# neoyinyao/Recommender

Hardware: AMD Instinct MI355X
Metric: examples/sec fwd+bwd, Criteo-DLRM 26×40M×128 batch 65536, 1/2/4/8 GPU (higher is better)
Workload: dtype fp32; 1 GPU; dlrm_criteo_26x40000000x128; global_batch=65536, per_gpu_batch=65536, rows=40000000, dim=128, slots=26, optimizer=sgd, parallelism=single, prefetch=False

## Files before the change

### recommender_amd/csrc/interaction.hip

```cpp
#include <map>
#include <mutex>
#include <tuple>
#include <type_traits>

#include "dlrm_shared.hpp"
#include "mfma_x3.hpp"

namespace rs {

struct InterMode {
  int self_interaction;
  int skip_gather;
};

__device__ __forceinline__ bool keep_pair(int i, int j, int self_i) {
  return self_i ? (i >= j) : (i < j);
}

struct GatherSrc {
  const float* table;
  int64_t n_rows;
  const void* ids;
  int32_t id_dtype;
  int32_t n_slots;
// ... 406 lines not shown
  const float* cur = row_of(first, raw_id(first));
  int64_t id_next = raw_id(first + 1);
#pragma unroll
  for (int s = 0; s < KS; ++s) load_rows(cur, s);
  load_g(first, lane);
  float* gs = gsm[wave];
  if (lane == 0) gs[ZS] = 0.f;
  for (int64_t b = first; b < last; ++b) {
    int lanev;
    asm volatile("v_mbcnt_lo_u32_b32 %0, -1, 0\n\tv_mbcnt_hi_u32_b32 %0, -1, %0" : "=v"(lanev));
    const int r = lanev & 31, h = lanev >> 5;
#pragma unroll
    for (int j = 0; j < GREG; ++j) gs[lane + 64 * j] = gnx[j];
    const float* nxt = row_of(b + 1, id_next);
    id_next = raw_id(b + 2);
    __builtin_amdgcn_s_waitcnt(0xc07f);
    __builtin_amdgcn_wave_barrier();
    float sa[KS];
#pragma unroll
    for (int s = 0; s < KS; ++s) {
      const int k = 2 * s + h;
      const bool in = r < F && k < F;
      const bool p1 = in && keep_pair(r, k, SELF);
      const bool p2 = in && keep_pair(k, r, SELF);
      const int j1 = p1 ? (SKIP ? r * F + k : compact_index(r, k, F, SELF)) : ZS;
      const int j2 = p2 ? (SKIP ? k * F + r : compact_index(k, r, F, SELF)) : ZS;
      sa[s] = gs[j1] + gs[j2];
    }
    f32x16 acc[NTILE];
#pragma unroll
    for (int c = 0; c < NTILE; ++c)
#pragma unroll
      for (int e = 0; e < 16; ++e) acc[c][e] = 0.f;
#pragma unroll
    for (int s = 0; s < KS; ++s) {
#pragma unroll
      for (int c = 0; c < NTILE; ++c)
        acc[c] = __builtin_amdgcn_mfma_f32_32x32x2f32(sa[s], xv[s][c], acc[c], 0, 0, 0);
    }
    __builtin_amdgcn_sched_barrier(0);
#pragma unroll
    for (int s = 0; s < KS; ++s) load_rows(nxt, s);
    __builtin_amdgcn_sched_barrier(0);
    float dpass[NTILE];
#pragma unroll
    for (int c = 0; c < NTILE; ++c) dpass[c] = gs[nz + NTILE * r + c];
    load_g(b + 1, lanev);
#pragma unroll
    for (int reg = 0; reg < 16; ++reg) {
      const int i = (reg & 3) + 8 * (reg >> 2) + 4 * h;
      if (i < F) {
        float v[NTILE];
#pragma unroll
        for (int c = 0; c < NTILE; ++c) v[c] = acc[c][reg] + (i == S ? dpass[c] : 0.f);
        float* dst = (i < S ? gemb + (b * S + i) * (int64_t)D : gdense + b * D) + NTILE * r;
        *reinterpret_cast<float4*>(dst) = make_float4(v[0], v[1], v[2], v[3]);
      }
    }
  }
  if (__any(oob) && lane == 0) flag_oob(src.err_flag);
}

constexpr int kDxLdx = 136;
constexpr int kDxRows = 28;
constexpr int kDxZt = 32 * 33;

template <bool ID64>
__global__ __launch_bounds__(256) void dlrm_fwd_dx_pipe(GatherSrc src, int64_t batch, int F,
                                                        float* __restrict__ out,
                                                        int64_t out_stride, FwdHead hd, int epw) {
  constexpr int D = 128, NT = 8;
  __shared__ __attribute__((aligned(16))) float lds[4][kDxRows * kDxLdx + kDxZt];
  const int wave = threadIdx.x >> 6, lane = threadIdx.x & 63;
  const int64_t first = ((int64_t)blockIdx.x * 4 + wave) * epw;
  if (first >= batch) return;
  const int64_t last = first + epw < batch ? first + epw : batch;
  const int r = lane & 15, g = lane >> 4;
  const int r32 = lane & 31, h = lane >> 5;
  const int S = src.n_slots;
  const int nzc = F * (F - 1) / 2;
  float* X = lds[wave];
  float(*z)[33] = reinterpret_cast<float(*)[33]>(lds[wave] + kDxRows * kDxLdx);
  float qz[8], qd[2], sa[2][8], qdn[4];
#pragma unroll
  for (int t = 0; t < 8; ++t) qz[t] = lane + 64 * t < nzc ? hd.q[lane + 64 * t] : 0.f;
#pragma unroll
  for (int t = 0; t < 2; ++t) qd[t] = hd.q[nzc + lane + 64 * t];
  const float cc = hd.c[0];
#pragma unroll
  for (int ib = 0; ib < 2; ++ib)
#pragma unroll
    for (int kk = 0; kk < 8; ++kk) {
      const int m = 16 * ib + r, k = 4 * kk + g;
      const bool in = m < F && k < F && m != k;
      const float v = hd.q[in ? compact_index(m < k ? m : k, m < k ? k : m, F, 0) : 0];
      sa[ib][kk] = in ? v : 0.f;
    }
#pragma unroll
  for (int c = 0; c < 4; ++c) qdn[c] = hd.q[nzc + 4 * r32 + c];
  int zoff[8];
#pragma unroll
  for (int t = 0; t < 8; ++t) {
    const int o = lane + 64 * t;
    int i = 0, j = 0;
    if (o < nzc) compact_pair(o, F, false, i, j);
    zoff[t] = o < nzc ? i * 33 + j : -1;
  }
  int64_t lo = 0, n_ok = src.n_rows;
  if (lane < S && src.slot_offsets) {
    lo = src.slot_offsets[lane];
    n_ok = src.slot_offsets[lane + 1] - lo;
  }
  bool oob = false;
  auto raw_id = [&](int64_t b) -> int64_t {
    const int64_t bb = b < last ? b : first;
    const int ln = lane < S ? lane : S - 1;
    const int64_t v = ID64 ? static_cast<const int64_t*>(src.ids)[bb * S + ln]
                           : static_cast<int64_t>(static_cast<const int32_t*>(src.ids)[bb * S + ln]);
    return lane < S ? v : 0;
  };
  auto row_of = [&](int64_t b, int64_t id) -> const float* {
    const bool live = b < last;
    const bool id_ok = id >= 0 && id < n_ok;
    if (lane < S && !id_ok && live) oob = true;
    if (lane < S) return id_ok ? src.table + (lo + id) * D : kZeroRow;
    return (lane == S && live) ? src.dense + (b < last ? b : first) * D : kZeroRow;
  };
  f4 a0[NT], a1[NT];
  float dnv[2];
  auto gather = [&](const float* mine, int64_t b) {
    const float* p0 = shfl_ptr(mine, r);
    const float* p1 = shfl_ptr(mine, 16 + r);
#pragma unroll
    for (int t = 0; t < NT; ++t) {
      a0[t] = *(gfloatx4*)(p0 + 4 * g + 16 * t);
      a1[t] = *(gfloatx4*)(p1 + 4 * g + 16 * t);
    }
    const int64_t bb = b < last ? b : first;
#pragma unroll
    for (int t = 0; t < 2; ++t) dnv[t] = *(gfloat*)(src.dense + bb * D + lane + 64 * t);
  };
  gather(row_of(first, raw_id(first)), first);
  int64_t id_next = raw_id(first + 1);
  for (int64_t b = first; b < last; ++b) {
    int lanev;
    asm volatile("v_mbcnt_lo_u32_b32 %0, -1, 0\n\tv_mbcnt_hi_u32_b32 %0, -1, %0" : "=v"(lanev));
    const int r = lanev & 15, g = (lanev >> 4) & 3;
    const int r32 = lanev & 31, h = (lanev >> 5) & 1;
    const float* nxt = row_of(b + 1, id_next);
    id_next = raw_id(b + 2);
    f4 c00 = {0.f, 0.f, 0.f, 0.f}, c01 = c00, c11 = c00;
#pragma unroll
    for (int t = 0; t < NT; ++t) {
#pragma unroll
      for (int c = 0; c < 4; ++c) {
        c00 = __builtin_amdgcn_mfma_f32_16x16x4f32(a0[t][c], a0[t][c], c00, 0, 0, 0);
        c01 = __builtin_amdgcn_mfma_f32_16x16x4f32(a0[t][c], a1[t][c], c01, 0, 0, 0);
        c11 = __builtin_amdgcn_mfma_f32_16x16x4f32(a1[t][c], a1[t][c], c11, 0, 0, 0);
      }
    }
#pragma unroll
    for (int t = 0; t < NT; ++t) {
      *reinterpret_cast<f4*>(&X[r * kDxLdx + 16 * t + 4 * g]) = a0[t];
      if (16 + r < kDxRows) *reinterpret_cast<f4*>(&X[(16 + r) * kDxLdx + 16 * t + 4 * g]) = a1[t];
    }
    float dn_cur[2] = {dnv[0], dnv[1]};
    __builtin_amdgcn_sched_barrier(0);
    gather(nxt, b + 1);
    __builtin_amdgcn_sched_barrier(0);
#pragma unroll
    for (int reg = 0; reg < 4; ++reg) {
      const int i = 4 * g + reg;
      z[i][r] = c00[reg];
      z[i][16 + r] = c01[reg];
      z[16 + r][i] = c01[reg];
      z[16 + i][16 + r] = c11[reg];
    }
    __builtin_amdgcn_wave_barrier();
    float* orow = out + b * out_stride;
    float hacc = 0.f;
    const int pad = nzc + D;
#pragma unroll
    for (int t = 0; t < 8; ++t) {
      const int o = lanev + 64 * t;
      const bool in = zoff[t] >= 0;
      const float v = in ? (&z[0][0])[zoff[t]] : 0.f;
      orow[in ? o : pad] = v;
      hacc += v * qz[t];
    }
    float* od = orow + nzc;
#pragma unroll
    for (int t = 0; t < 2; ++t) {
      const int d = lanev + 64 * t;
      od[d] = dn_cur[t];
      hacc += dn_cur[t] * qd[t];
    }
#pragma unroll
    for (int off = 32; off > 0; off >>= 1) hacc += __shfl_xor(hacc, off);
    {
      const float v = hacc + cc;
      hd.y[b] = hd.act == 2 ? 1.f / (1.f + expf(-v)) : (hd.act == 1 ? fmaxf(v, 0.f) : v);
    }
    {
      const int o = pad + lanev;
      orow[o < out_stride ? o : pad] = 0.f;
    }
#pragma unroll
    for (int t = 0; t < NT; ++t) {
      constexpr int KK = kDxRows / 4;
      float bv[KK];
#pragma unroll
      for (int kk = 0; kk < KK; ++kk) bv[kk] = X[(4 * kk + g) * kDxLdx + 16 * t + r];
      f4 d0 = {0.f, 0.f, 0.f, 0.f}, d1 = d0;
#pragma unroll
      for (int kk = 0; kk < KK; ++kk) {
        d0 = __builtin_amdgcn_mfma_f32_16x16x4f32(sa[0][kk], bv[kk], d0, 0, 0, 0);
        d1 = __builtin_amdgcn_mfma_f32_16x16x4f32(sa[1][kk], bv[kk], d1, 0, 0, 0);
      }
#pragma unroll
      for (int reg = 0; reg < 4; ++reg) {
        const int i0 = 4 * g + reg, i1 = 16 + 4 * g + reg;
        X[i0 * kDxLdx + 16 * t + r] = d0[reg];
        if (i1 < kDxRows) X[i1 * kDxLdx + 16 * t + r] = d1[reg];
      }
    }
    __builtin_amdgcn_wave_barrier();
    float* de = hd.dxu_emb + b * S * (int64_t)D;
#pragma unroll
    for (int s2 = 0; s2 < kDxRows / 2; ++s2) {
      const int i = 2 * s2 + h < S ? 2 * s2 + h : S;
      f4 v = *reinterpret_cast<const f4*>(&X[i * kDxLdx + 4 * r32]);
      const bool emb = i < S;
#pragma unroll
      for (int c = 0; c < 4; ++c) v[c] = emb ? v[c] : v[c] + qdn[c];
      float* dst = emb ? de + i * D : hd.dxu_dense + b * D;
      *reinterpret_cast<f4*>(dst + 4 * r32) = v;
    }
    __builtin_amdgcn_wave_barrier();
  }
  if (__any(oob) && lane == 0) flag_oob(src.err_flag);
}

__device__ __forceinline__ void split3(const f4& lo, const f4& hi, bf8& h, bf8& m,
                                       bf8& l) {
#pragma unroll
  for (int j = 0; j < 4; ++j) {
    bf2 hp, mp, lp;
    split_pair(j < 2 ? f2{lo[2 * j], lo[2 * j + 1]} : f2{hi[2 * j - 4], hi[2 * j - 3]}, hp, mp, lp);
    h[2 * j] = hp[0];
    h[2 * j + 1] = hp[1];
    m[2 * j] = mp[0];
    m[2 * j + 1] = mp[1];
    l[2 * j] = lp[0];
    l[2 * j + 1] = lp[1];
  }
}

constexpr int kTrainAtop = 512;
constexpr int kTrainNI = 13;
template <int D>
constexpr int train_m() { return kTrainAtop + 2 + kTrainNI * D + D; }
constexpr int kTrainM = train_m<128>();

struct TrainArgs {
  const float* q;
  const float* c;
  const float* label;
  const float* xin;
  float eps;
  float gscale;
  float* y;
  float* grad_emb;
  float* part;
};

typedef short shortx4 __attribute__((ext_vector_type(4)));
typedef short shortx8 __attribute__((ext_vector_type(8)));
typedef __attribute__((address_space(3))) shortx4 lds_shortx4;

__device__ __forceinline__ f4 mfma6_xs(const bf8& xh, const bf8& xm, const bf8& xl,
                                            const bf8& sh, const bf8& sm, const bf8& sl,
                                            f4 c) {
  c = __builtin_amdgcn_mfma_f32_16x16x32_bf16(xm, sm, c, 0, 0, 0);
  c = __builtin_amdgcn_mfma_f32_16x16x32_bf16(xl, sh, c, 0, 0, 0);
  c = __builtin_amdgcn_mfma_f32_16x16x32_bf16(xh, sl, c, 0, 0, 0);
  c = __builtin_amdgcn_mfma_f32_16x16x32_bf16(xm, sh, c, 0, 0, 0);
  c = __builtin_amdgcn_mfma_f32_16x16x32_bf16(xh, sm, c, 0, 0, 0);
  return __builtin_amdgcn_mfma_f32_16x16x32_bf16(xh, sh, c, 0, 0, 0);
}

constexpr int kChPlane = 32 * 32 * 2;
constexpr int kChImage = 3 * kChPlane;
__device__ __forceinline__ int ch_off(int row, int col) {
  const int chunk = (col >> 3) ^ ((row >> 1) & 3) ^ (((row >> 3) & 1) << 1);
  return row * 64 + 16 * chunk + 2 * (col & 7);
}
constexpr int kChStageLd = 36;
template <int D>
constexpr int chunk_region_floats() {
  return (kChImage / 4 + 32 * kChStageLd + D) > train_m<D>() ? (kChImage / 4 + 32 * kChStageLd + D)
                                                             : train_m<D>();
}

template <int D, bool ID64>
__global__ __launch_bounds__(256, 2) void dlrm_train_chunk(GatherSrc src, int64_t batch, int F,
                                                        TrainArgs ta, float* g_rows, int epw) {
  static_assert(D == 64 || D == 128, "train kernel laid out for D = 64 or 128");
  constexpr int NT = D / 16, NC = D / 32, DL = D / 4, RPI = 64 / DL, DPL = D / 64;
  constexpr int TM = train_m<D>();
  constexpr int RW = chunk_region_floats<D>();
  __shared__ __attribute__((aligned(16))) float lds[4][RW];
  __shared__ __attribute__((aligned(16))) float qlane[64][12];
  __shared__ __attribute__((aligned(16))) float qsh[kTrainAtop];
  __shared__ __attribute__((aligned(16))) bf8 sash[2][3][64];
  const int wave = threadIdx.x >> 6, lane = threadIdx.x & 63;
  const int64_t first = ((int64_t)blockIdx.x * 4 + wave) * epw;
  const int64_t last = first + epw < batch ? first + epw : batch;
  const bool active = first < batch;
  const int r = lane & 15, g = lane >> 4;
  const int S = src.n_slots;
  const int nzc = F * (F - 1) / 2;
  char* img = reinterpret_cast<char*>(lds[wave]);
  float* stg = lds[wave] + kChImage / 4;
  float* ubot = stg + 32 * kChStageLd;
  for (int e = threadIdx.x; e < kTrainAtop; e += 256) {
    const float v = ta.q[e < nzc + D ? e : 0];
    qsh[e] = e < nzc + D ? v : 0.f;
  }
  if (wave == 0) {
    float qv[12];
    bool qk[12];
#pragma unroll
    for (int reg = 0; reg < 4; ++reg) {
      const int i0 = 4 * g + reg, j0 = r;
      const int i1 = 4 * g + reg, j1 = 16 + r;
      const int i2 = 16 + 4 * g + reg, j2 = 16 + r;
      qk[reg] = i0 < j0 && j0 < F;
      qk[4 + reg] = j1 < F;
      qk[8 + reg] = i2 < j2 && j2 < F;
      qv[reg] = ta.q[qk[reg] ? compact_index(i0, j0, F, 0) : 0];
      qv[4 + reg] = ta.q[qk[4 + reg] ? compact_index(i1, j1, F, 0) : 0];
      qv[8 + reg] = ta.q[qk[8 + reg] ? compact_index(i2, j2, F, 0) : 0];
    }
#pragma unroll
    for (int k = 0; k < 12; ++k) qlane[lane][k] = qk[k] ? qv[k] : 0.f;
  }
  if (wave == 1) {
#pragma unroll
    for (int ib = 0; ib < 2; ++ib) {
      f4 v[2];
#pragma unroll
      for (int j = 0; j < 8; ++j) {
        const int m = 16 * ib + r, kk = 8 * g + j;
        const bool in = m < F && kk < F && m != kk;
        const float q = ta.q[in ? compact_index(m < kk ? m : kk, m < kk ? kk : m, F, 0) : 0];
        v[j >> 2][j & 3] = in ? q : 0.f;
      }
      split3(v[0], v[1], sash[ib][0][lane], sash[ib][1][lane], sash[ib][2][lane]);
    }
  }
  __syncthreads();
  const float cc = ta.c[0];
  float az[12], ad[4], abot[DPL][kTrainNI], sbot[DPL];
  float s_top = 0.f, loss = 0.f;
#pragma unroll
  for (int k = 0; k < 12; ++k) az[k] = 0.f;
#pragma unroll
  for (int k = 0; k < 4; ++k) ad[k] = 0.f;
#pragma unroll
  for (int k = 0; k < DPL; ++k) {
    sbot[k] = 0.f;
#pragma unroll
    for (int i = 0; i < kTrainNI; ++i) abot[k][i] = 0.f;
  }
  int64_t lo = 0, n_ok = src.n_rows;
  if (lane < S && src.slot_offsets) {
    lo = src.slot_offsets[lane];
    n_ok = src.slot_offsets[lane + 1] - lo;
  }
  bool oob = false;
  auto raw_id = [&](int64_t b) -> int64_t {
    const int64_t bb = b < last ? b : first;
    const int ln = lane < S ? lane : S - 1;
    const int64_t v = ID64 ? static_cast<const int64_t*>(src.ids)[bb * S + ln]
                           : static_cast<int64_t>(static_cast<const int32_t*>(src.ids)[bb * S + ln]);
    return lane < S ? v : 0;
  };
  auto row_of = [&](int64_t b, int64_t id) -> const float* {
    const bool live = b < last;
    const bool id_ok = id >= 0 && id < n_ok;
    if (lane < S && !id_ok && live) oob = true;
    if (lane < S) return id_ok ? src.table + (lo + id) * D : kZeroRow;
    return (lane == S && live) ? src.dense + (b < last ? b : first) * D : kZeroRow;
  };
  f4 a0[NT], a1[NT];
  f4 dn4;
  const float* p0 = nullptr;
  const float* p1 = nullptr;
  auto load_chunk = [&](int s) {
    a0[2 * s] = *(gfloatx4*)(p0 + 32 * s + 8 * g);
    a0[2 * s + 1] = *(gfloatx4*)(p0 + 32 * s + 8 * g + 4);
    a1[2 * s] = *(gfloatx4*)(p1 + 32 * s + 8 * g);
    a1[2 * s + 1] = *(gfloatx4*)(p1 + 32 * s + 8 * g + 4);
  };
  auto load_side = [&](int64_t b) {
    const int cl = lane & (DL - 1);
    const int64_t bb = b < last ? b : first;
    dn4 = *(gfloatx4*)(src.dense + bb * D + 4 * cl);
  };
  if (active) {
    {
      const float* mine = row_of(first, raw_id(first));
      p0 = shfl_ptr(mine, r);
      p1 = shfl_ptr(mine, 16 + r);
      load_side(first);
#pragma unroll
      for (int s = 0; s < NC; ++s) load_chunk(s);
    }
    int64_t id_next = raw_id(first + 1);
    for (int64_t b = first; b < last; ++b) {
      int lanev;
      asm volatile("v_mbcnt_lo_u32_b32 %0, -1, 0\n\tv_mbcnt_hi_u32_b32 %0, -1, %0" : "=v"(lanev));
      const int r = lanev & 15, g = (lanev >> 4) & 3;
      {
        const float* nxt = row_of(b + 1, id_next);
        p0 = shfl_ptr(nxt, r);
        p1 = shfl_ptr(nxt, 16 + r);
      }
      id_next = raw_id(b + 2);
      const f4 dn = dn4;
      float xb[kTrainNI];
      typedef __attribute__((address_space(4))) const float cfloat;
      const int bq = __builtin_amdgcn_readfirstlane((int)b);
      const cfloat* xr = (const cfloat*)(ta.xin + (int64_t)bq * kTrainNI);
#pragma unroll
      for (int i = 0; i < kTrainNI; ++i) xb[i] = xr[i];
      const float lb = ((const cfloat*)ta.label)[bq];
      load_side(b + 1);
      float* de = ta.grad_emb + b * S * (int64_t)D;
      f4 c00 = {0.f, 0.f, 0.f, 0.f}, c01 = c00, c11 = c00;
      const int q = (lanev >> 2) & 3, p4 = lanev & 3;
#pragma unroll
      for (int s = 0; s < NC; ++s) {
        bf8 sa[2][3];
#pragma unroll
        for (int ib = 0; ib < 2; ++ib)
#pragma unroll
          for (int pt = 0; pt < 3; ++pt) sa[ib][pt] = sash[ib][pt][lanev & 63];
        bf8 h0, m0, l0, h1, m1, l1;
        split3(a0[2 * s], a0[2 * s + 1], h0, m0, l0);
        split3(a1[2 * s], a1[2 * s + 1], h1, m1, l1);
        __builtin_amdgcn_sched_barrier(0);
        load_chunk(s);
        __builtin_amdgcn_sched_barrier(0);
        c00 = mfma6(h0, m0, l0, h0, m0, l0, c00);
        c01 = mfma6(h0, m0, l0, h1, m1, l1, c01);
        c11 = mfma6(h1, m1, l1, h1, m1, l1, c11);
        *reinterpret_cast<bf8*>(img + 0 * kChPlane + ch_off(r, 8 * g)) = h0;
        *reinterpret_cast<bf8*>(img + 1 * kChPlane + ch_off(r, 8 * g)) = m0;
        *reinterpret_cast<bf8*>(img + 2 * kChPlane + ch_off(r, 8 * g)) = l0;
        *reinterpret_cast<bf8*>(img + 0 * kChPlane + ch_off(16 + r, 8 * g)) = h1;
        *reinterpret_cast<bf8*>(img + 1 * kChPlane + ch_off(16 + r, 8 * g)) = m1;
        *reinterpret_cast<bf8*>(img + 2 * kChPlane + ch_off(16 + r, 8 * g)) = l1;
        __builtin_amdgcn_wave_barrier();
#pragma unroll
        for (int tt = 0; tt < 2; ++tt) {
          bf8 xp[3];
#pragma unroll
          for (int pt = 0; pt < 3; ++pt) {
            const int o0 = pt * kChPlane + ch_off(8 * g + q, 16 * tt + 4 * p4);
            const int o1 = pt * kChPlane + ch_off(8 * g + 4 + q, 16 * tt + 4 * p4);
            const shortx4 lo4 =
                __builtin_amdgcn_ds_read_tr16_b64_v4i16((lds_shortx4*)(img + o0));
            const shortx4 hi4 =
                __builtin_amdgcn_ds_read_tr16_b64_v4i16((lds_shortx4*)(img + o1));
            const shortx8 v8 = __builtin_shufflevector(lo4, hi4, 0, 1, 2, 3, 4, 5, 6, 7);
            xp[pt] = __builtin_bit_cast(bf8, v8);
          }
          f4 d0 = {0.f, 0.f, 0.f, 0.f}, d1 = d0;
          d0 = mfma6_xs(xp[0], xp[1], xp[2], sa[0][0], sa[0][1], sa[0][2], d0);
          d1 = mfma6_xs(xp[0], xp[1], xp[2], sa[1][0], sa[1][1], sa[1][2], d1);
          const int col = 16 * tt + 4 * g;
          *reinterpret_cast<f4*>(stg + r * kChStageLd + col) = d0;
          *reinterpret_cast<f4*>(stg + (16 + r) * kChStageLd + col) = d1;
          if (r == S) *reinterpret_cast<f4*>(ubot + 32 * s + col) = d0;
          if (16 + r == S) *reinterpret_cast<f4*>(ubot + 32 * s + col) = d1;
        }
        __builtin_amdgcn_wave_barrier();
#pragma unroll
        for (int pp = 0; pp < 4; ++pp) {
          const int i = 8 * pp + (lanev >> 3), c8 = lanev & 7;
          const f4 v = *reinterpret_cast<const f4*>(stg + i * kChStageLd + 4 * c8);
          if (i < S)
            __builtin_nontemporal_store(v, reinterpret_cast<f4*>(de + i * D + 32 * s + 4 * c8));
        }
        __builtin_amdgcn_wave_barrier();
      }
      const int cl = lanev & (DL - 1), rg = (lanev / DL) & (RPI - 1);
      float zr[12];
#pragma unroll
      for (int reg = 0; reg < 4; ++reg) {
        zr[reg] = c00[reg];
        zr[4 + reg] = c01[reg];
        zr[8 + reg] = c11[reg];
      }
      float hacc = 0.f;
      {
        const f4* ql = reinterpret_cast<const f4*>(&qlane[lanev & 63][0]);
#pragma unroll
        for (int q4 = 0; q4 < 3; ++q4) {
          const f4 qv = ql[q4];
#pragma unroll
          for (int k = 0; k < 4; ++k) hacc += zr[4 * q4 + k] * qv[k];
        }
        const f4 qd = *reinterpret_cast<const f4*>(&qsh[nzc + 4 * cl]);
        if (rg == 0) {
#pragma unroll
          for (int k = 0; k < 4; ++k) hacc += dn[k] * qd[k];
        }
      }
      hacc = wave_sum(hacc);
      const float p = 1.f / (1.f + expf(-(hacc + cc)));
      {
        const float pc = fminf(fmaxf(p, ta.eps), 1.f - ta.eps);
        loss += -(lb * logf(pc + ta.eps) + (1.f - lb) * logf((1.f - pc) + ta.eps));
      }
      const bool inside = p >= ta.eps && p <= 1.f - ta.eps;
      const float pcg = fminf(fmaxf(p, ta.eps), 1.f - ta.eps);
      const float dbce = -(lb / (pcg + ta.eps)) + (1.f - lb) / ((1.f - pcg) + ta.eps);
      const float dp = inside ? ta.gscale * dbce : 0.f;
      const float G = dp * (p * (1.f - p));
      if (lanev == 0) {
        ta.y[b] = p;
        g_rows[b] = G;
      }
      s_top += G;
#pragma unroll
      for (int k = 0; k < 12; ++k) az[k] += zr[k] * G;
#pragma unroll
      for (int k = 0; k < 4; ++k) ad[k] += dn[k] * G;
      {
        const f4 v = *reinterpret_cast<const f4*>(ubot + 4 * cl);
        const f4 qdn = *reinterpret_cast<const f4*>(&qsh[nzc + 4 * cl]);
#pragma unroll
        for (int k = 0; k < DPL; ++k) {
          const int c = DPL * rg + k;
          const float gd = __fmul_rn(G, v[c] + qdn[c]);
          const float gb = dn[c] > 0.f ? gd : 0.f;
          sbot[k] += gb;
#pragma unroll
          for (int ii = 0; ii < kTrainNI; ++ii) abot[k][ii] += xb[ii] * gb;
        }
      }
      __builtin_amdgcn_wave_barrier();
    }
  }
  __syncthreads();
  float* X = lds[wave];
  for (int e = lane; e < TM; e += 64) X[e] = 0.f;
  __builtin_amdgcn_wave_barrier();
  if (active) {
    const int cl = lane & (DL - 1), rg = lane / DL;
#pragma unroll
    for (int reg = 0; reg < 4; ++reg) {
      const int i0 = 4 * g + reg, j0 = r, i1 = 4 * g + reg, j1 = 16 + r, i2 = 16 + 4 * g + reg, j2 = 16 + r;
      if (i0 < j0 && j0 < F) X[compact_index(i0, j0, F, 0)] = az[reg];
      if (j1 < F) X[compact_index(i1, j1, F, 0)] = az[4 + reg];
      if (i2 < j2 && j2 < F) X[compact_index(i2, j2, F, 0)] = az[8 + reg];
    }
    if (rg == 0) {
#pragma unroll
      for (int k = 0; k < 4; ++k) X[nzc + 4 * cl + k] = ad[k];
    }
    if (lane == 0) {
      X[kTrainAtop] = s_top;
      X[kTrainAtop + 1] = loss;
    }
#pragma unroll
    for (int k = 0; k < DPL; ++k) {
      const int d = 4 * cl + DPL * rg + k;
#pragma unroll
      for (int ii = 0; ii < kTrainNI; ++ii) X[kTrainAtop + 2 + ii * D + d] = abot[k][ii];
      X[kTrainAtop + 2 + kTrainNI * D + d] = sbot[k];
    }
  }
  __syncthreads();
  for (int e = threadIdx.x; e < TM; e += 256) {
    float v = lds[0][e];
    v += lds[1][e];
    v += lds[2][e];
    v += lds[3][e];
    ta.part[(int64_t)blockIdx.x * TM + e] = v;
  }
  if (__any(oob) && lane == 0) flag_oob(src.err_flag);
}


template <int GREG, int KS, bool ID64>
static void launch_pipe_t(const GatherSrc& src, int64_t batch, int F, InterMode md,
                          const float* gout, int64_t gstride, float* gemb, float* gdense, int,
                          hipStream_t st, const float* gscale = nullptr) {
  auto go = [&](auto kern) {
    const int epw = pipe_epw(reinterpret_cast<const void*>(kern), batch);
    kern<<<ceil_div(batch, 4 * (int64_t)epw), 256, 0, st>>>(src, batch, F, gout, gstride, gemb,
                                                           gdense, epw, gscale);
  };
  if (gscale) {
    go(dlrm_bwd_pipe<128, GREG, KS, false, false, ID64, true>);
    return;
  }
  if (md.self_interaction) {
    if (md.skip_gather) go(dlrm_bwd_pipe<128, GREG, KS, true, true, ID64>);
    else go(dlrm_bwd_pipe<128, GREG, KS, true, false, ID64>);
  } else {
    if (md.skip_gather) go(dlrm_bwd_pipe<128, GREG, KS, false, true, ID64>);
    else go(dlrm_bwd_pipe<128, GREG, KS, false, false, ID64>);
  }
}

template <int GREG, int KS>
static void launch_pipe(const GatherSrc& src, int64_t batch, int F, InterMode md,
                        const float* gout, int64_t gstride, float* gemb, float* gdense, int epw,
                        hipStream_t st, const float* gscale = nullptr) {
  if (src.id_dtype == RS_ID_I64)
    launch_pipe_t<GREG, KS, true>(src, batch, F, md, gout, gstride, gemb, gdense, epw, st, gscale);
  else
    launch_pipe_t<GREG, KS, false>(src, batch, F, md, gout, gstride, gemb, gdense, epw, st, gscale);
}

template <class Src, bool DLRM_OUT>
__global__ __launch_bounds__(64) void inter_fwd_generic(Src src, int64_t batch, int F, int D,
                                                        InterMode md, float* __restrict__ out,
                                                        int64_t out_stride) {
  extern __shared__ __attribute__((aligned(16))) float xs[];
  const int lane = threadIdx.x;
  const int64_t b = blockIdx.x;
  const int ld = D + 1;
  bool oob = false;
  for (int i = 0; i < F; ++i) {
    const float* xr = src.row(b, i, D, oob);
    for (int d = lane; d < D; d += 64) xs[i * ld + d] = xr ? xr[d] : 0.f;
  }
  __syncthreads();
  float* orow = out + b * out_stride;
  for (int o = lane; o < F * F; o += 64) {
    int i = o / F, j = o - i * F;
    bool keep = keep_pair(i, j, md.self_interaction);
    if (!keep && !md.skip_gather) continue;
    float s = 0.f;
    if (keep)
      for (int d = 0; d < D; ++d) s = fmaf(xs[i * ld + d], xs[j * ld + d], s);
    if (md.skip_gather)
      orow[o] = s;
    else
      orow[compact_index(i, j, F, md.self_interaction)] = s;
  }
  if constexpr (DLRM_OUT) {
    const int nz = out_width(F, md.self_interaction, md.skip_gather);
    float* od = orow + nz;
    for (int d = lane; d < D; d += 64) od[d] = src.dense[b * D + d];
    for (int64_t o = nz + D + lane; o < out_stride; o += 64) orow[o] = 0.f;
    if (__any(oob) && lane == 0) flag_oob(src.err_flag);
  }
}

template <class Src, bool DLRM_OUT>
__global__ __launch_bounds__(64) void inter_bwd_generic(Src src, int64_t batch, int F, int D,
                                                        InterMode md, const float* __restrict__ gout,
                                                        int64_t gstride, float* __restrict__ gx,
                                                        float* __restrict__ gemb,
                                                        float* __restrict__ gdense) {
  extern __shared__ __attribute__((aligned(16))) float sm[];
  float* xs = sm;
  float* ss = sm + F * (D + 1);
  const int lane = threadIdx.x;
  const int64_t b = blockIdx.x;
  const int ld = D + 1, ls = F + 1;
  bool oob = false;
  const float* grow = gout + b * gstride;
  for (int i = 0; i < F; ++i) {
    const float* xr = src.row(b, i, D, oob);
    for (int d = lane; d < D; d += 64) xs[i * ld + d] = xr ? xr[d] : 0.f;
  }
  for (int o = lane; o < F * F; o += 64) {
    int i = o / F, k = o - i * F;
    float v = 0.f;
    if (keep_pair(i, k, md.self_interaction))
      v += md.skip_gather ? grow[i * F + k] : grow[compact_index(i, k, F, md.self_interaction)];
    if (keep_pair(k, i, md.self_interaction))
      v += md.skip_gather ? grow[k * F + i] : grow[compact_index(k, i, F, md.self_interaction)];
    ss[i * ls + k] = v;
  }
  __syncthreads();
  for (int o = lane; o < F * D; o += 64) {
    int i = o / D, d = o - i * D;
    float s = 0.f;
    for (int k = 0; k < F; ++k) s = fmaf(ss[i * ls + k], xs[k * ld + d], s);
    if constexpr (DLRM_OUT) {
      if (i < src.n_slots) {
        gemb[(b * src.n_slots + i) * (int64_t)D + d] = s;
      } else {
        gdense[b * D + d] = s + grow[out_width(F, md.self_interaction, md.skip_gather) + d];
      }
    } else {
      gx[(b * F + i) * (int64_t)D + d] = s;
    }
  }
}

__global__ __launch_bounds__(256) void fm_fwd_kernel(const float* __restrict__ emb, int64_t batch,
                                                     int F, int D, float* __restrict__ out) {
  const int wave = threadIdx.x >> 6, lane = threadIdx.x & 63;
  const int64_t b = (int64_t)blockIdx.x * 4 + wave;
  if (b >= batch) return;
  const float* e = emb + b * F * (int64_t)D;
  float part = 0.f;
  for (int d = lane; d < D; d += 64) {
    float s = 0.f, q = 0.f;
    for (int f = 0; f < F; ++f) {
      float x = e[f * D + d];
      s += x;
      q += x * x;
    }
    part += s * s - q;
  }
  for (int off = 32; off > 0; off >>= 1) part += __shfl_down(part, off);
  if (lane == 0) out[b] = 0.5f * part;
}

__global__ __launch_bounds__(256) void fm_bwd_kernel(const float* __restrict__ emb,
                                                     const float* __restrict__ gout, int64_t batch,
                                                     int F, int D, float* __restrict__ gemb) {
  const int wave = threadIdx.x >> 6, lane = threadIdx.x & 63;
  const int64_t b = (int64_t)blockIdx.x * 4 + wave;
  if (b >= batch) return;
  const float* e = emb + b * F * (int64_t)D;
  float* ge = gemb + b * F * (int64_t)D;
  const float g = gout[b];
  for (int d = lane; d < D; d += 64) {
    float s = 0.f;
    for (int f = 0; f < F; ++f) s += e[f * D + d];
    for (int f = 0; f < F; ++f) ge[f * D + d] = g * (s - e[f * D + d]);
  }
}

template <class Src, bool DLRM_OUT>
static int32_t launch_fwd(const Src& src, int64_t batch, int F, int D, InterMode md, float* out,
                          int64_t out_stride, bool aligned16, hipStream_t st) {
  if (batch == 0) return RS_OK;
  if (F <= 32 && aligned16) {
    int64_t blocks = ceil_div(batch, 4);
    switch (D) {
      case 16: inter_fwd_mfma<16, Src, DLRM_OUT><<<blocks, 256, 0, st>>>(src, batch, F, md, out, out_stride); RS_CHECK_LAUNCH(); return RS_OK;
      case 32: inter_fwd_mfma<32, Src, DLRM_OUT><<<blocks, 256, 0, st>>>(src, batch, F, md, out, out_stride); RS_CHECK_LAUNCH(); return RS_OK;
      case 64: inter_fwd_mfma<64, Src, DLRM_OUT><<<blocks, 256, 0, st>>>(src, batch, F, md, out, out_stride); RS_CHECK_LAUNCH(); return RS_OK;
      case 128: inter_fwd_mfma<128, Src, DLRM_OUT><<<blocks, 256, 0, st>>>(src, batch, F, md, out, out_stride); RS_CHECK_LAUNCH(); return RS_OK;
      case 256: inter_fwd_mfma<256, Src, DLRM_OUT><<<blocks, 256, 0, st>>>(src, batch, F, md, out, out_stride); RS_CHECK_LAUNCH(); return RS_OK;
      default: break;
    }
  }
  size_t lds = (size_t)F * (D + 1) * 4;
  if (lds > 64 * 1024) {
    set_error("interaction F=%d D=%d too large for the generic kernel", F, D);
    return RS_E_UNSUPPORTED;
  }
  inter_fwd_generic<Src, DLRM_OUT><<<batch, 64, lds, st>>>(src, batch, F, D, md, out, out_stride);
  RS_CHECK_LAUNCH();
  return RS_OK;
}

template <class Src, bool DLRM_OUT>
static int32_t launch_bwd(const Src& src, int64_t batch, int F, int D, InterMode md,
                          const float* gout, int64_t gstride, float* gx, float* gemb, float* gdense,
                          bool aligned16, hipStream_t st) {
  if (batch == 0) return RS_OK;
  if constexpr (DLRM_OUT && std::is_same<Src, GatherSrc>::value) {
    const int epw = kPipeEPW;
    const int gw = out_width(F, md.self_interaction, md.skip_gather) + D;
    if (F <= 32 && aligned16 && D == 128 && gw <= 20 * 64) {
      const bool k14 = F <= 28;
      if (gw <= 8 * 64) {
        if (k14) launch_pipe<8, 14>(src, batch, F, md, gout, gstride, gemb, gdense, epw, st);
        else launch_pipe<8, 16>(src, batch, F, md, gout, gstride, gemb, gdense, epw, st);
        RS_CHECK_LAUNCH();
        return RS_OK;
      }
      {
        if (k14) launch_pipe<20, 14>(src, batch, F, md, gout, gstride, gemb, gdense, epw, st);
        else launch_pipe<20, 16>(src, batch, F, md, gout, gstride, gemb, gdense, epw, st);
        RS_CHECK_LAUNCH();
        return RS_OK;
      }
    }
  }
  if (F <= 32 && aligned16) {
    int64_t blocks = ceil_div(batch, 4);
    switch (D) {
      case 32: inter_bwd_mfma<32, Src, DLRM_OUT><<<blocks, 256, 0, st>>>(src, batch, F, md, gout, gstride, gx, gemb, gdense); RS_CHECK_LAUNCH(); return RS_OK;
      case 64: inter_bwd_mfma<64, Src, DLRM_OUT><<<blocks, 256, 0, st>>>(src, batch, F, md, gout, gstride, gx, gemb, gdense); RS_CHECK_LAUNCH(); return RS_OK;
      case 128: inter_bwd_mfma<128, Src, DLRM_OUT><<<blocks, 256, 0, st>>>(src, batch, F, md, gout, gstride, gx, gemb, gdense); RS_CHECK_LAUNCH(); return RS_OK;
      default: break;
    }
  }
  size_t lds = ((size_t)F * (D + 1) + (size_t)F * (F + 1)) * 4;
  if (lds > 64 * 1024) {
    set_error("interaction F=%d D=%d too large for the generic kernel", F, D);
    return RS_E_UNSUPPORTED;
  }
  inter_bwd_generic<Src, DLRM_OUT><<<batch, 64, lds, st>>>(src, batch, F, D, md, gout, gstride, gx,
                                                           gemb, gdense);
  RS_CHECK_LAUNCH();
  return RS_OK;
}

static bool al16(const void* p) { return (reinterpret_cast<uintptr_t>(p) & 15) == 0; }

}

using namespace rs;

extern "C" int32_t rs_dot_interaction_fwd(const float* x, int64_t batch, int32_t F, int32_t D,
                                          int32_t self_interaction, int32_t skip_gather, float* out,
                                          int64_t out_stride, void* stream) {
  RS_CHECK_ARG(F >= 1 && D >= 1 && batch >= 0, "bad sizes");
  RS_CHECK_ARG(out_stride >= out_width(F, self_interaction, skip_gather), "out_stride too small");
  RS_CHECK_ARG(batch == 0 || (x && out), "null pointer");
  DenseSrc src{x, F};
  return launch_fwd<DenseSrc, false>(src, batch, F, D, {self_interaction, skip_gather}, out,
                                     out_stride, al16(x), as_stream(stream));
}

extern "C" int32_t rs_dot_interaction_bwd(const float* x, const float* grad_out, int64_t batch,
                                          int32_t F, int32_t D, int32_t self_interaction,
                                          int32_t skip_gather, int64_t grad_stride, float* grad_x,
                                          void* stream) {
  RS_CHECK_ARG(F >= 1 && D >= 1 && batch >= 0, "bad sizes");
  RS_CHECK_ARG(grad_stride >= out_width(F, self_interaction, skip_gather), "grad_stride too small");
  RS_CHECK_ARG(batch == 0 || (x && grad_out && grad_x), "null pointer");
  DenseSrc src{x, F};
  return launch_bwd<DenseSrc, false>(src, batch, F, D, {self_interaction, skip_gather}, grad_out,
                                     grad_stride, grad_x, nullptr, nullptr, al16(x) && al16(grad_x),
                                     as_stream(stream));
}

extern "C" int32_t rs_dlrm_interaction_fwd(const float* table, int64_t n_rows, int32_t D,
                                           const void* ids, int32_t id_dtype, int32_t n_slots,
                                           const int64_t* slot_offsets, const float* dense,
                                           int64_t batch, int32_t compact, float* out,
                                           int64_t out_stride, int32_t* err_flag, void* stream) {
  const int F = n_slots + 1;
  const InterMode md{0, compact ? 0 : 1};
  RS_CHECK_ARG(n_slots >= 1 && D >= 1 && batch >= 0, "bad sizes");
  RS_CHECK_ARG(id_dtype == RS_ID_I32 || id_dtype == RS_ID_I64, "bad id dtype");
  RS_CHECK_ARG(out_stride >= out_width(F, 0, md.skip_gather) + D, "out_stride too small");
  RS_CHECK_ARG(batch == 0 || (table && ids && dense && out), "null pointer");
  GatherSrc src{table, n_rows, ids, id_dtype, n_slots, slot_offsets, dense, err_flag};
  return launch_fwd<GatherSrc, true>(src, batch, F, D, md, out, out_stride,
                                     al16(table) && al16(dense), as_stream(stream));
}

extern "C" int32_t rs_dlrm_interaction_bwd(const float* table, int64_t n_rows, int32_t D,
                                           const void* ids, int32_t id_dtype, int32_t n_slots,
                                           const int64_t* slot_offsets, const float* dense,
                                           int64_t batch, int32_t compact, const float* grad_out,
                                           int64_t grad_stride, float* grad_emb, float* grad_dense,
                                           void* stream) {
  const int F = n_slots + 1;
  const InterMode md{0, compact ? 0 : 1};
  RS_CHECK_ARG(n_slots >= 1 && D >= 1 && batch >= 0, "bad sizes");
  RS_CHECK_ARG(grad_stride >= out_width(F, 0, md.skip_gather) + D, "grad_stride too small");
  RS_CHECK_ARG(batch == 0 || (table && ids && dense && grad_out && grad_emb && grad_dense),
               "null pointer");
  GatherSrc src{table, n_rows, ids, id_dtype, n_slots, slot_offsets, dense, nullptr};
  return launch_bwd<GatherSrc, true>(src, batch, F, D, md, grad_out, grad_stride, nullptr,
                                     grad_emb, grad_dense,
                                     al16(table) && al16(dense) && al16(grad_emb) && al16(grad_dense),
                                     as_stream(stream));
}

extern "C" int32_t rs_dlrm_interaction_bwd_rank1(const float* table, int64_t n_rows, int32_t D,
                                                 const void* ids, int32_t id_dtype,
                                                 int32_t n_slots, const int64_t* slot_offsets,
                                                 const float* dense, int64_t batch,
                                                 const float* gscale, const float* grad_row,
                                                 int64_t width, float* grad_emb,
                                                 float* grad_dense, void* stream) {
  const int F = n_slots + 1;
  const InterMode md{0, 0};
  const int gw = out_width(F, 0, 0) + D;
  RS_CHECK_ARG(n_slots >= 1 && D >= 1 && batch >= 0, "bad sizes");
  RS_CHECK_ARG(width >= gw, "width too small");
  if (batch == 0) return RS_OK;
  RS_CHECK_ARG(table && ids && dense && gscale && grad_row && grad_emb && grad_dense,
               "null pointer");
  if (!(F <= 32 && D == 128 && gw <= 20 * 64 && al16(table) && al16(dense) && al16(grad_emb) &&
        al16(grad_dense))) {
    set_error("rs_dlrm_interaction_bwd_rank1: needs D = 128, F <= 32, 16-B aligned buffers");
    return RS_E_UNSUPPORTED;
  }
  GatherSrc src{table, n_rows, ids, id_dtype, n_slots, slot_offsets, dense, nullptr};
  hipStream_t st = as_stream(stream);
  const bool k14 = F <= 28;
  if (gw <= 8 * 64) {
    if (k14) launch_pipe<8, 14>(src, batch, F, md, grad_row, width, grad_emb, grad_dense, 0, st, gscale);
    else launch_pipe<8, 16>(src, batch, F, md, grad_row, width, grad_emb, grad_dense, 0, st, gscale);
  } else {
    if (k14) launch_pipe<20, 14>(src, batch, F, md, grad_row, width, grad_emb, grad_dense, 0, st, gscale);
    else launch_pipe<20, 16>(src, batch, F, md, grad_row, width, grad_emb, grad_dense, 0, st, gscale);
  }
  RS_CHECK_LAUNCH();
  return RS_OK;
}

extern "C" int32_t rs_fm_fwd(const float* emb, int64_t batch, int32_t F, int32_t D, float* out,
                             void* stream) {
  RS_CHECK_ARG(F >= 1 && D >= 1 && batch >= 0, "bad sizes");
  if (batch == 0) return RS_OK;
  RS_CHECK_ARG(emb && out, "null pointer");
  fm_fwd_kernel<<<ceil_div(batch, 4), 256, 0, as_stream(stream)>>>(emb, batch, F, D, out);
  RS_CHECK_LAUNCH();
  return RS_OK;
}

extern "C" int32_t rs_fm_bwd(const float* emb, const float* grad_out, int64_t batch, int32_t F,
                             int32_t D, float* grad_emb, void* stream) {
  RS_CHECK_ARG(F >= 1 && D >= 1 && batch >= 0, "bad sizes");
  if (batch == 0) return RS_OK;
  RS_CHECK_ARG(emb && grad_out && grad_emb, "null pointer");
  fm_bwd_kernel<<<ceil_div(batch, 4), 256, 0, as_stream(stream)>>>(emb, grad_out, batch, F, D,
                                                                   grad_emb);
  RS_CHECK_LAUNCH();
  return RS_OK;
}

extern "C" int32_t rs_dlrm_interaction_fwd_head(const float* table, int64_t n_rows, int32_t D,
                                                const void* ids, int32_t id_dtype,
                                                int32_t n_slots, const int64_t* slot_offsets,
                                                const float* dense, int64_t batch, float* out,
                                                int64_t out_stride, const float* q,
                                                const float* c, int32_t act, float* y,
                                                int32_t* err_flag, void* stream) {
  const int F = n_slots + 1;
  const InterMode md{0, 0};
  RS_CHECK_ARG(n_slots >= 1 && F <= 32 && D == 128 && batch >= 0,
               "rs_dlrm_interaction_fwd_head: needs D = 128 and at most 31 slots");
  RS_CHECK_ARG(id_dtype == RS_ID_I32 || id_dtype == RS_ID_I64, "bad id dtype");
  RS_CHECK_ARG(out_stride >= out_width(F, 0, 0) + D, "out_stride too small");
  RS_CHECK_ARG(act >= 0 && act <= 2, "bad activation");
  RS_CHECK_ARG(batch == 0 || (table && ids && dense && out && q && c && y), "null pointer");
  RS_CHECK_ARG(al16(table) && al16(dense), "table and dense must be 16-byte aligned");
  if (batch == 0) return RS_OK;
  GatherSrc src{table, n_rows, ids, id_dtype, n_slots, slot_offsets, dense, err_flag};
  FwdHead hd{q, c, y, act};
  inter_fwd_mfma<128, GatherSrc, true, true>
      <<<ceil_div(batch, 4), 256, 0, as_stream(stream)>>>(src, batch, F, md, out, out_stride, hd);
  RS_CHECK_LAUNCH();
  return RS_OK;
}

extern "C" int32_t rs_dlrm_interaction_fwd_head_dx(const float* table, int64_t n_rows, int32_t D,
                                                   const void* ids, int32_t id_dtype,
                                                   int32_t n_slots, const int64_t* slot_offsets,
                                                   const float* dense, int64_t batch, float* out,
                                                   int64_t out_stride, const float* q,
                                                   const float* c, int32_t act, float* y,
                                                   float* dxu_emb, float* dxu_dense,
                                                   int32_t* err_flag, void* stream) {
  const int F = n_slots + 1;
  const InterMode md{0, 0};
  RS_CHECK_ARG(n_slots >= 1 && F <= 32 && D == 128 && batch >= 0,
               "rs_dlrm_interaction_fwd_head_dx: needs D = 128 and at most 31 slots");
  RS_CHECK_ARG(id_dtype == RS_ID_I32 || id_dtype == RS_ID_I64, "bad id dtype");
  RS_CHECK_ARG(out_stride >= out_width(F, 0, 0) + D, "out_stride too small");
  RS_CHECK_ARG(act >= 0 && act <= 2, "bad activation");
  RS_CHECK_ARG(batch == 0 || (table && ids && dense && out && q && c && y && dxu_emb && dxu_dense),
               "null pointer");
  RS_CHECK_ARG(al16(table) && al16(dense), "table and dense must be 16-byte aligned");
  if (batch == 0) return RS_OK;
  GatherSrc src{table, n_rows, ids, id_dtype, n_slots, slot_offsets, dense, err_flag};
  FwdHead hd{q, c, y, act, dxu_emb, dxu_dense};
  hipStream_t st = as_stream(stream);
  if (F <= kDxRows && out_stride > out_width(F, 0, 0) + D &&
      out_stride <= out_width(F, 0, 0) + D + 64) {
    auto go = [&](auto kern) {
      const int epw = pipe_epw(reinterpret_cast<const void*>(kern), batch);
      kern<<<ceil_div(batch, 4 * (int64_t)epw), 256, 0, st>>>(src, batch, F, out, out_stride, hd, epw);
    };
    if (id_dtype == RS_ID_I64) go(dlrm_fwd_dx_pipe<true>);
    else go(dlrm_fwd_dx_pipe<false>);
  } else {
    inter_fwd_mfma<128, GatherSrc, true, true, true>
        <<<ceil_div(batch, 4), 256, 0, st>>>(src, batch, F, md, out, out_stride, hd);
  }
  RS_CHECK_LAUNCH();
  return RS_OK;
}

extern "C" size_t rs_dlrm_train_workspace_size(int64_t batch) {
  return (size_t)(ceil_div(batch, 4) + 32) * kTrainM * sizeof(float) + 256;
}

static int64_t train_blocks(int64_t batch, int32_t D, int id_dtype) {
  const void* k = D == 128 ? (id_dtype == RS_ID_I64 ? reinterpret_cast<const void*>(dlrm_train_chunk<128, true>)
                                                    : reinterpret_cast<const void*>(dlrm_train_chunk<128, false>))
                           : (id_dtype == RS_ID_I64 ? reinterpret_cast<const void*>(dlrm_train_chunk<64, true>)
                                                    : reinterpret_cast<const void*>(dlrm_train_chunk<64, false>));
  return ceil_div(batch, 4 * (int64_t)pipe_epw(k, batch, 1));
}

static int32_t train_step_launch(
    const float* table, int64_t n_rows, int32_t D, const void* ids, int32_t id_dtype,
    int32_t n_slots, const int64_t* slot_offsets, const float* dense, const float* xin,
    int32_t n_in, const float* label, int64_t batch, const float* q, const float* c, float eps,
    float loss_scale, float* y, float* grad_emb, float* sums, void* workspace, size_t ws_bytes,
    int32_t* err_flag, void* stream, float* g_rows, bool fold = true) {
  const int F = n_slots + 1;
  RS_CHECK_ARG((D == 128 || D == 64) && n_slots >= 1 && F <= kDxRows && n_in == kTrainNI &&
                   batch >= 1,
               "rs_dlrm_train_step_fwd_unit: needs D = 128 or 64, at most %d slots, %d dense inputs",
               kDxRows - 1, kTrainNI);
  RS_CHECK_ARG(id_dtype == RS_ID_I32 || id_dtype == RS_ID_I64, "bad id dtype");
  RS_CHECK_ARG(loss_scale > 0.f, "loss_scale must be positive");
  RS_CHECK_ARG(table && ids && dense && xin && label && q && c && y && grad_emb && sums && workspace,
               "null pointer");
  RS_CHECK_ARG(al16(table) && al16(dense) && al16(grad_emb), "table, dense and grad rows must be 16-byte aligned");
  RS_CHECK_ARG(ws_bytes >= rs_dlrm_train_workspace_size(batch), "workspace too small");
  hipStream_t st = as_stream(stream);
  GatherSrc src{table, n_rows, ids, id_dtype, n_slots, slot_offsets, dense, err_flag};
  float* part = static_cast<float*>(workspace);
  TrainArgs ta{q, c, label, xin, eps, loss_scale, y, grad_emb, part};
  int64_t blocks = 0;
  auto go = [&](auto kern) {
    const int epw = pipe_epw(reinterpret_cast<const void*>(kern), batch, 1);
    blocks = ceil_div(batch, 4 * (int64_t)epw);
    kern<<<blocks, 256, 0, st>>>(src, batch, F, ta, g_rows, epw);
  };
  if (D == 128) {
    if (id_dtype == RS_ID_I64) go(dlrm_train_chunk<128, true>);
    else go(dlrm_train_chunk<128, false>);
  } else {
    if (id_dtype == RS_ID_I64) go(dlrm_train_chunk<64, true>);
    else go(dlrm_train_chunk<64, false>);
  }
  RS_CHECK_LAUNCH();
  if (!fold) return RS_OK;
  const int tm = D == 128 ? train_m<128>() : train_m<64>();
  return fold_two_level(part, (int)blocks, tm, part + (size_t)blocks * tm, sums, st);
}

extern "C" int32_t rs_dlrm_train_step_fwd_unit(
    const float* table, int64_t n_rows, int32_t D, const void* ids, int32_t id_dtype,
    int32_t n_slots, const int64_t* slot_offsets, const float* dense, const float* xin,
    int32_t n_in, const float* label, int64_t batch, const float* q, const float* c, float eps,
    float loss_scale, float* y, float* unit_rows, float* g_rows, float* sums, void* workspace,
    size_t ws_bytes, int32_t* err_flag, void* stream) {
  RS_CHECK_ARG(g_rows, "null pointer");
  return train_step_launch(table, n_rows, D, ids, id_dtype, n_slots, slot_offsets, dense, xin,
                           n_in, label, batch, q, c, eps, loss_scale, y, unit_rows, sums,
                           workspace, ws_bytes, err_flag, stream, g_rows);
}

extern "C" int32_t rs_dlrm_train_step_fwd_unit_nofold(
    const float* table, int64_t n_rows, int32_t D, const void* ids, int32_t id_dtype,
    int32_t n_slots, const int64_t* slot_offsets, const float* dense, const float* xin,
    int32_t n_in, const float* label, int64_t batch, const float* q, const float* c, float eps,
    float loss_scale, float* y, float* unit_rows, float* g_rows, void* workspace,
    size_t ws_bytes, int32_t* err_flag, void* stream) {
  RS_CHECK_ARG(g_rows, "null pointer");
  float dummy_sums[1];
  return train_step_launch(table, n_rows, D, ids, id_dtype, n_slots, slot_offsets, dense, xin,
                           n_in, label, batch, q, c, eps, loss_scale, y, unit_rows, dummy_sums,
                           workspace, ws_bytes, err_flag, stream, g_rows, false);
}

extern "C" int32_t rs_dlrm_train_fold(const void* workspace, size_t ws_bytes, int64_t batch,
                                      int32_t D, int32_t id_dtype, float* sums, void* stream) {
  RS_CHECK_ARG((D == 128 || D == 64) && batch >= 1, "rs_dlrm_train_fold: D = 128 or 64, batch >= 1");
  RS_CHECK_ARG(id_dtype == RS_ID_I32 || id_dtype == RS_ID_I64, "bad id dtype");
  RS_CHECK_ARG(workspace && sums, "null pointer");
  RS_CHECK_ARG(ws_bytes >= rs_dlrm_train_workspace_size(batch), "workspace too small");
  const int64_t blocks = train_blocks(batch, D, id_dtype);
  const int tm = D == 128 ? train_m<128>() : train_m<64>();
  float* part = static_cast<float*>(const_cast<void*>(workspace));
  return fold_two_level(part, (int)blocks, tm, part + (size_t)blocks * tm, sums, as_stream(stream));
}
```

Measured before the change: 105.4 million examples/sec.

## Specialize train kernel on slot count and coalesce tail-row gradient stores via LDS strip

Adds a TAIL template parameter so the slot count (24+TAIL) is a compile-time constant. This removes the per-row predicate on gradient stores. The tail rows beyond 24 are staged into an extra LDS strip per wave and written out fully coalesced after all chunks, instead of as partially masked 8-lane stores per chunk. It also inserts a full waitcnt before the main loop and lets all lanes store y/g_rows. The cost is more LDS per block, which can affect occupancy, plus extra template instantiations.

```diff
diff --git a/recommender_amd/csrc/interaction.hip b/recommender_amd/csrc/interaction.hip
--- a/recommender_amd/csrc/interaction.hip
+++ b/recommender_amd/csrc/interaction.hip
@@ -732,14 +732,16 @@
                                                              : train_m<D>();
 }
 
-template <int D, bool ID64>
+template <int D, bool ID64, int TAIL = -1>
 __global__ __launch_bounds__(256, 2) void dlrm_train_chunk(GatherSrc src, int64_t batch, int F,
                                                         TrainArgs ta, float* g_rows, int epw) {
   static_assert(D == 64 || D == 128, "train kernel laid out for D = 64 or 128");
+  static_assert(TAIL >= -1 && 24 + TAIL < kDxRows, "S = 24 + TAIL slots and the dense row");
   constexpr int NT = D / 16, NC = D / 32, DL = D / 4, RPI = 64 / DL, DPL = D / 64;
   constexpr int TM = train_m<D>();
   constexpr int RW = chunk_region_floats<D>();
-  __shared__ __attribute__((aligned(16))) float lds[4][RW];
+  constexpr int STRIP = TAIL > 0 ? TAIL * D : 0;
+  __shared__ __attribute__((aligned(16))) float lds[4][RW + STRIP];
   __shared__ __attribute__((aligned(16))) float qlane[64][12];
   __shared__ __attribute__((aligned(16))) float qsh[kTrainAtop];
   __shared__ __attribute__((aligned(16))) bf8 sash[2][3][64];
@@ -748,11 +750,12 @@
   const int64_t last = first + epw < batch ? first + epw : batch;
   const bool active = first < batch;
   const int r = lane & 15, g = lane >> 4;
-  const int S = src.n_slots;
+  const int S = TAIL >= 0 ? 24 + TAIL : src.n_slots;
   const int nzc = F * (F - 1) / 2;
   char* img = reinterpret_cast<char*>(lds[wave]);
   float* stg = lds[wave] + kChImage / 4;
   float* ubot = stg + 32 * kChStageLd;
+  float* strip = lds[wave] + RW;
   for (int e = threadIdx.x; e < kTrainAtop; e += 256) {
     const float v = ta.q[e < nzc + D ? e : 0];
     qsh[e] = e < nzc + D ? v : 0.f;
@@ -848,6 +851,11 @@
       for (int s = 0; s < NC; ++s) load_chunk(s);
     }
     int64_t id_next = raw_id(first + 1);
+    if constexpr (TAIL >= 0) {
+      __builtin_amdgcn_sched_barrier(0);
+      __builtin_amdgcn_s_waitcnt(0x0F70);
+      __builtin_amdgcn_sched_barrier(0);
+    }
     for (int64_t b = first; b < last; ++b) {
       int lanev;
       asm volatile("v_mbcnt_lo_u32_b32 %0, -1, 0\n\tv_mbcnt_hi_u32_b32 %0, -1, %0" : "=v"(lanev));
@@ -917,14 +925,37 @@
           if (16 + r == S) *reinterpret_cast<f4*>(ubot + 32 * s + col) = d1;
         }
         __builtin_amdgcn_wave_barrier();
-#pragma unroll
-        for (int pp = 0; pp < 4; ++pp) {
-          const int i = 8 * pp + (lanev >> 3), c8 = lanev & 7;
-          const f4 v = *reinterpret_cast<const f4*>(stg + i * kChStageLd + 4 * c8);
-          if (i < S)
+        if constexpr (TAIL >= 0) {
+#pragma unroll
+          for (int pp = 0; pp < 3; ++pp) {
+            const int i = 8 * pp + (lanev >> 3), c8 = lanev & 7;
+            const f4 v = *reinterpret_cast<const f4*>(stg + i * kChStageLd + 4 * c8);
             __builtin_nontemporal_store(v, reinterpret_cast<f4*>(de + i * D + 32 * s + 4 * c8));
+          }
+          if constexpr (TAIL > 0) {
+            const int t = (lanev >> 3) < TAIL - 1 ? (lanev >> 3) : TAIL - 1, c8 = lanev & 7;
+            const f4 v = *reinterpret_cast<const f4*>(stg + (24 + t) * kChStageLd + 4 * c8);
+            *reinterpret_cast<f4*>(strip + t * D + 32 * s + 4 * c8) = v;
+          }
+        } else {
+#pragma unroll
+          for (int pp = 0; pp < 4; ++pp) {
+            const int i = 8 * pp + (lanev >> 3), c8 = lanev & 7;
+            const f4 v = *reinterpret_cast<const f4*>(stg + i * kChStageLd + 4 * c8);
+            if (i < S)
+              __builtin_nontemporal_store(v, reinterpret_cast<f4*>(de + i * D + 32 * s + 4 * c8));
+          }
         }
         __builtin_amdgcn_wave_barrier();
+      }
+      if constexpr (TAIL > 0) {
+#pragma unroll
+        for (int k = 0; k < (TAIL * DL + 63) / 64; ++k) {
+          const int w = 64 * k + (lanev & 63);
+          const int t = w / DL < TAIL - 1 ? w / DL : TAIL - 1, c = w & (DL - 1);
+          const f4 v = *reinterpret_cast<const f4*>(strip + t * D + 4 * c);
+          __builtin_nontemporal_store(v, reinterpret_cast<f4*>(de + (24 + t) * D + 4 * c));
+        }
       }
       const int cl = lanev & (DL - 1), rg = (lanev / DL) & (RPI - 1);
       float zr[12];
@@ -960,7 +991,10 @@
       const float dbce = -(lb / (pcg + ta.eps)) + (1.f - lb) / ((1.f - pcg) + ta.eps);
       const float dp = inside ? ta.gscale * dbce : 0.f;
       const float G = dp * (p * (1.f - p));
-      if (lanev == 0) {
+      if constexpr (TAIL >= 0) {
+        ta.y[b] = p;
+        g_rows[b] = G;
+      } else if (lanev == 0) {
         ta.y[b] = p;
         g_rows[b] = G;
       }
@@ -1430,12 +1464,16 @@
   return (size_t)(ceil_div(batch, 4) + 32) * kTrainM * sizeof(float) + 256;
 }
 
-static int64_t train_blocks(int64_t batch, int32_t D, int id_dtype) {
+static int train_epw(int64_t batch, int32_t D, int id_dtype) {
   const void* k = D == 128 ? (id_dtype == RS_ID_I64 ? reinterpret_cast<const void*>(dlrm_train_chunk<128, true>)
                                                     : reinterpret_cast<const void*>(dlrm_train_chunk<128, false>))
                            : (id_dtype == RS_ID_I64 ? reinterpret_cast<const void*>(dlrm_train_chunk<64, true>)
                                                     : reinterpret_cast<const void*>(dlrm_train_chunk<64, false>));
-  return ceil_div(batch, 4 * (int64_t)pipe_epw(k, batch, 1));
+  return pipe_epw(k, batch, 1);
+}
+
+static int64_t train_blocks(int64_t batch, int32_t D, int id_dtype) {
+  return ceil_div(batch, 4 * (int64_t)train_epw(batch, D, id_dtype));
 }
 
 static int32_t train_step_launch(
@@ -1459,19 +1497,24 @@
   GatherSrc src{table, n_rows, ids, id_dtype, n_slots, slot_offsets, dense, err_flag};
   float* part = static_cast<float*>(workspace);
   TrainArgs ta{q, c, label, xin, eps, loss_scale, y, grad_emb, part};
-  int64_t blocks = 0;
-  auto go = [&](auto kern) {
-    const int epw = pipe_epw(reinterpret_cast<const void*>(kern), batch, 1);
-    blocks = ceil_div(batch, 4 * (int64_t)epw);
-    kern<<<blocks, 256, 0, st>>>(src, batch, F, ta, g_rows, epw);
+  const int epw = train_epw(batch, D, id_dtype);
+  const int64_t blocks = ceil_div(batch, 4 * (int64_t)epw);
+  auto go = [&](auto kern) { kern<<<blocks, 256, 0, st>>>(src, batch, F, ta, g_rows, epw); };
+  auto by_ids = [&](auto d, auto tail) {
+    if (id_dtype == RS_ID_I64) go(dlrm_train_chunk<decltype(d)::value, true, decltype(tail)::value>);
+    else go(dlrm_train_chunk<decltype(d)::value, false, decltype(tail)::value>);
   };
-  if (D == 128) {
-    if (id_dtype == RS_ID_I64) go(dlrm_train_chunk<128, true>);
-    else go(dlrm_train_chunk<128, false>);
-  } else {
-    if (id_dtype == RS_ID_I64) go(dlrm_train_chunk<64, true>);
-    else go(dlrm_train_chunk<64, false>);
-  }
+  auto by_tail = [&](auto d) {
+    switch (n_slots - 24) {
+      case 0: return by_ids(d, std::integral_constant<int, 0>());
+      case 1: return by_ids(d, std::integral_constant<int, 1>());
+      case 2: return by_ids(d, std::integral_constant<int, 2>());
+      case 3: return by_ids(d, std::integral_constant<int, 3>());
+    }
+    by_ids(d, std::integral_constant<int, -1>());
+  };
+  if (D == 128) by_tail(std::integral_constant<int, 128>());
+  else by_tail(std::integral_constant<int, 64>());
   RS_CHECK_LAUNCH();
   if (!fold) return RS_OK;
   const int tm = D == 128 ? train_m<128>() : train_m<64>();
```

New measurement: 104.8 million examples/sec. Within noise of the previous version (-0.6%).
